# jzr99/Geo4D

Hardware: AMD Instinct MI355X
Metric: denoised latent frames/sec (16x320x512, 50-step DDIM) (higher is better)
Workload: dtype bf16x3m

## Files before the change

### geo4d_amd/_lib.py

```python
import ctypes as C
import os

import torch

_HERE = os.path.dirname(os.path.abspath(__file__))
LIB_PATH = os.environ.get("GEO4D_HIP_LIB") or os.path.join(_HERE, "csrc", "libgeo4d_hip.so")
ABI_VERSION = 9

F32, BF16, F16, BF16X3, F16X2 = 0, 1, 2, 3, 4


class Geo4DNativeError(RuntimeError):
    pass


class ConvGemm(C.Structure):
    _fields_ = [
        ("A", C.c_void_p), ("W", C.c_void_p), ("O", C.c_void_p),
        ("bias", C.c_void_p), ("rowbias", C.c_void_p), ("R", C.c_void_p),
        ("zeros", C.c_void_p), ("workspace", C.c_void_p), ("workspace_bytes", C.c_size_t),
        ("lda", C.c_long), ("ldw", C.c_long), ("ldo", C.c_long), ("ldr", C.c_long), ("ldrb", C.c_long),
        ("a_bs", C.c_long), ("w_bs", C.c_long), ("o_bs", C.c_long), ("r_bs", C.c_long),
        ("M", C.c_int), ("N", C.c_int), ("K", C.c_int), ("batch", C.c_int),
        ("Cin", C.c_int),
# ... 6 lines not shown
        ("a_split", C.c_int), ("w_split", C.c_int), ("o_split", C.c_int), ("gn_colsum", C.c_void_p), ("sat_count", C.c_void_p),
    ]


class GroupNorm(C.Structure):
    _fields_ = [
        ("x", C.c_void_p), ("y", C.c_void_p), ("gamma", C.c_void_p), ("beta", C.c_void_p),
        ("workspace", C.c_void_p), ("workspace_bytes", C.c_size_t),
        ("ldx", C.c_long), ("ldy", C.c_long),
        ("F", C.c_int), ("HW", C.c_int), ("C", C.c_int), ("groups", C.c_int), ("frames_per_stat", C.c_int),
        ("act", C.c_int), ("dtype", C.c_int), ("eps", C.c_float), ("colsum", C.c_void_p), ("split_out", C.c_int), ("colsum_rows", C.c_int),
        ("sat_count", C.c_void_p),
    ]


class Attention(C.Structure):
    _fields_ = [
        ("q", C.c_void_p), ("o", C.c_void_p),
        ("k", C.c_void_p * 2), ("vt", C.c_void_p * 2), ("zeros", C.c_void_p),
        ("ldq", C.c_long), ("ldo", C.c_long), ("ldk", C.c_long * 2), ("ldvt", C.c_long * 2), ("vt_bs", C.c_long * 2),
        ("Nk", C.c_int * 2), ("kv_div", C.c_int * 2),
        ("B", C.c_int), ("H", C.c_int), ("Nq", C.c_int), ("nseg", C.c_int), ("head_dim", C.c_int), ("dtype", C.c_int),
        ("scale", C.c_float), ("split_out", C.c_int), ("variant", C.c_int), ("qkv_split", C.c_int),
    ]


class Align(C.Structure):
    _fields_ = [
        ("pred", C.c_void_p), ("conf", C.c_void_p), ("logdepth", C.c_void_p), ("cams", C.c_void_p), ("slot_trf", C.c_void_p),
        ("slot_ptr", C.c_void_p), ("slot_idx", C.c_void_p),
# ... 16 lines not shown
        ("slot_st", C.c_void_p), ("s_depth", C.c_void_p), ("t_depth", C.c_void_p), ("depth_ok", C.c_void_p),
        ("traj", C.c_void_p), ("traj_align", C.c_void_p), ("traj_valid", C.c_void_p), ("slot_img", C.c_void_p), ("img_slot_ptr", C.c_void_p),
        ("img_slot_idx", C.c_void_p), ("grad_traj", C.c_void_p),
        ("n_imgs", C.c_int), ("n_groups", C.c_int), ("n_slots", C.c_int), ("slots_per_group", C.c_int), ("n_listed_slots", C.c_int),
        ("n_focals", C.c_int), ("norm_pw_scale", C.c_int),
        ("focal_break", C.c_float), ("base_scale", C.c_float), ("ppx", C.c_float), ("ppy", C.c_float), ("smooth_weight", C.c_float),
        ("translation_weight", C.c_float), ("traj_weight", C.c_float),
    ]


SIGNATURES = {
    "geo4d_conv_gemm": (C.c_int, [C.POINTER(ConvGemm), C.c_void_p]),
    "geo4d_conv_gemm_colsum_rows": (C.c_int, [C.POINTER(ConvGemm)]),
    "geo4d_groupnorm_workspace": (C.c_size_t, [C.c_int, C.c_int, C.c_int, C.c_int]),
    "geo4d_groupnorm": (C.c_int, [C.POINTER(GroupNorm), C.c_void_p]),
    "geo4d_layernorm": (C.c_int, [C.c_void_p, C.c_long, C.c_void_p, C.c_long, C.c_int, C.c_int, C.c_float, C.c_void_p,
                                  C.c_void_p, C.c_int, C.c_void_p]),
    "geo4d_layernorm_split": (C.c_int, [C.c_void_p, C.c_long, C.c_void_p, C.c_long, C.c_int, C.c_int, C.c_float, C.c_void_p,
                                        C.c_void_p, C.c_int, C.c_void_p, C.c_void_p]),
    "geo4d_softmax_rows": (C.c_int, [C.c_void_p, C.c_long, C.c_void_p, C.c_long, C.c_long, C.c_int, C.c_float, C.c_int,
                                     C.c_void_p]),
    "geo4d_softmax_rows_causal": (C.c_int, [C.c_void_p, C.c_long, C.c_void_p, C.c_long, C.c_long, C.c_int, C.c_float, C.c_int,
                                            C.c_int, C.c_void_p]),
    "geo4d_attention": (C.c_int, [C.POINTER(Attention), C.c_void_p]),
    "geo4d_temporal_attention": (C.c_int, [C.c_void_p, C.c_long, C.c_void_p, C.c_long, C.c_void_p, C.c_long, C.c_void_p,
                                           C.c_long, C.c_int, C.c_int, C.c_int, C.c_int, C.c_int, C.c_float, C.c_int,
                                           C.c_void_p]),
    "geo4d_temporal_attention2": (C.c_int, [C.c_void_p, C.c_long, C.c_void_p, C.c_long, C.c_void_p, C.c_long, C.c_void_p,
                                            C.c_long, C.c_int, C.c_int, C.c_int, C.c_int, C.c_int, C.c_float, C.c_int,
                                            C.c_int, C.c_void_p]),
# ... 98 lines not shown
```

### geo4d_amd/csrc/norm.hip

```cpp
#include <type_traits>
#include "common.h"
#include "geo4d_hip.h"

namespace {

__host__ __device__ inline int gn_rows_per_chunk(int HW, int F) {
    long r = ((long)HW * F + 1023) / 1024;
    r = (r + 3) / 4 * 4;
    if (r < 4) r = 4;
    if (r > 1024) r = 1024;
    return (int)r;
}

template <typename T>
__device__ __forceinline__ void gn_partial_body(char* smem, const T* __restrict__ x, long ldx, int HW, int C, int G,
                                                int R, int nchunk, float* __restrict__ part, int chunk, int f) {
    constexpr int EPC = Elem<T>::EPC;
    float* stage = (float*)smem;
    float* chs = stage + 256 * 2 * EPC;
    float* chq = chs + C;
    const int tid = threadIdx.x;
    const int CPR = C / EPC;
    const int TC = CPR < 256 ? CPR : 256;
    const int TR = 256 / TC;
// ... 124 lines not shown
    if (tid == 0) {
        s = ((red[0][0] + red[1][0]) + red[2][0]) + red[3][0];
        q = ((red[0][1] + red[1][1]) + red[2][1]) + red[3][1];
        const double n = (double)blocks_per_stat * rows * cpg;
        const double mean = s / n;
        double var = q / n - mean * mean;
        if (var < 0.0) var = 0.0;
        stats[((long)stat * G + grp) * 2 + 0] = (float)mean;
        stats[((long)stat * G + grp) * 2 + 1] = (float)(1.0 / sqrt(var + (double)eps));
    }
}

template <typename T, int SPLIT>
__device__ __forceinline__ void gn_apply_body(const T* __restrict__ x, long ldx, T* __restrict__ y, long ldy,
                                              int HW, int C, int G, int R, const float* st, const float* __restrict__ gamma,
                                              const float* __restrict__ beta, int act, int chunk, int f, unsigned long long* sat) {
    constexpr int EPC = Elem<T>::EPC;
    const int tid = threadIdx.x;
    const int CPR = C / EPC;
    const int TC = CPR < 256 ? CPR : 256;
    const int TR = 256 / TC;
    const int tc = tid % TC, tr = tid / TC;
    if (tr >= TR) return;
    const int row0 = chunk * R;
    const int rows = min(R, HW - row0);
    const int cpg = C / G;
    const T* xb = x + ((long)f * HW + row0) * ldx;
    T* yb = y + ((long)f * HW + row0) * ldy;
    for (int cc = tc; cc < CPR; cc += TC) {
        float sc[EPC], sh[EPC];
#pragma unroll
        for (int j = 0; j < EPC; ++j) {
            const int c = cc * EPC + j;
            const int gi = c / cpg;
            const float mean = st[gi * 2], rstd = st[gi * 2 + 1];
            sc[j] = rstd * gamma[c];
            sh[j] = beta[c] - mean * sc[j];
        }
        for (int r = tr; r < rows; r += 4 * TR) {
            u32x4 v[4];
#pragma unroll
            for (int u = 0; u < 4; ++u) {
                const int ru = r + u * TR;
                v[u] = ru < rows ? *(const u32x4*)(xb + (long)ru * ldx + cc * EPC) : u32x4{0u, 0u, 0u, 0u};
// ... 13 lines not shown
                if constexpr (SPLIT == 1) store_split4(yb + (long)ru * ldy, cc, e);
                else if constexpr (SPLIT == 2) {
                    count_f16_saturation(sat, e);
                    store4_f16((char*)y + ((long)f * HW + row0 + ru) * ldy * 2, cc, e);
                } else *(u32x4*)(yb + (long)ru * ldy + cc * EPC) = f32_to_chunk<T>(e);
            }
        }
    }
}
template <typename T, int SPLIT>
__global__ __launch_bounds__(256) void gn_apply_kernel(const T* __restrict__ x, long ldx, T* __restrict__ y, long ldy,
                                                       int HW, int C, int G, int fps, int R,
                                                       const float* __restrict__ stats, const float* __restrict__ gamma,
                                                       const float* __restrict__ beta, int act, unsigned long long* sat) {
    const int f = blockIdx.y;
    gn_apply_body<T, SPLIT>(x, ldx, y, ldy, HW, C, G, R, stats + (long)(f / fps) * G * 2, gamma, beta, act, blockIdx.x, f, sat);
}

template <typename T, int MAXC, int SPLIT = 0>
__global__ __launch_bounds__(256) void ln_kernel(const T* __restrict__ x, long ldx, T* __restrict__ y, long ldy, int M, int C,
                                                 float eps, const float* __restrict__ gamma, const float* __restrict__ beta, unsigned long long* sat) {
    constexpr int EPC = Elem<T>::EPC;
    const int lane = threadIdx.x & 63;
    const long row = (long)blockIdx.x * 4 + (threadIdx.x >> 6);
    if (row >= M) return;
    const int CPR = C / EPC;
    float e[MAXC][EPC];
    float s = 0.f;
#pragma unroll
    for (int i = 0; i < MAXC; ++i) {
        const int cc = lane + i * 64;
// ... 98 lines not shown
    m = wave_max(m);
    if ((tid & 63) == 0) red[tid >> 6] = m;
    __syncthreads();
    m = fmaxf(fmaxf(red[0], red[1]), fmaxf(red[2], red[3]));
    __syncthreads();
    float s = 0.f;
    for (int c = tid; c < cols; c += 256) s += __expf(xr[c] * scale - m);
    s = wave_sum(s);
    if ((tid & 63) == 0) red[tid >> 6] = s;
    __syncthreads();
    s = (red[0] + red[1]) + (red[2] + red[3]);
    const float inv = 1.0f / s;
    for (int c = tid; c < cols; c += 256) Elem<T>::st(yr + c, __expf(xr[c] * scale - m) * inv);
}

template <typename T, int SPLIT>
int groupnorm_typed(const geo4d_groupnorm_t& p, hipStream_t s) {
    constexpr int EPC = Elem<T>::EPC;
    int R = gn_rows_per_chunk(p.HW, p.F);
    int nchunk = (p.HW + R - 1) / R;
    float* part = (float*)p.workspace;
    const size_t smem = (size_t)256 * 2 * EPC * 4 + (size_t)2 * p.C * 4;
    const int nstat = p.F / p.frames_per_stat;
    float* stats = part + (size_t)p.F * nchunk * p.groups * 3;
    if (p.colsum) {
        const int crows = p.colsum_rows > 0 ? p.colsum_rows : 32;
        hipLaunchKernelGGL(gn_finalize_cols_kernel, dim3(nstat * p.groups), dim3(256), 0, s, p.colsum, (p.frames_per_stat * p.HW) / crows,
                           p.C, p.groups, p.eps, stats, nstat, crows);
        GEO4D_CHECK_LAUNCH();
    } else {
        hipLaunchKernelGGL(gn_partial_kernel<T>, dim3(nchunk, p.F), dim3(256), smem, s, (const T*)p.x, (long)p.ldx, p.HW, p.C, p.groups,
                           R, nchunk, part);
        GEO4D_CHECK_LAUNCH();
        hipLaunchKernelGGL(gn_finalize_kernel, dim3((nstat * p.groups + 3) / 4), dim3(256), 0, s, part, nchunk, p.frames_per_stat,
                           p.groups, p.eps, stats, nstat);
        GEO4D_CHECK_LAUNCH();
    }
    hipLaunchKernelGGL((gn_apply_kernel<T, SPLIT>), dim3(nchunk, p.F), dim3(256), 0, s, (const T*)p.x, (long)p.ldx, (T*)p.y, (long)p.ldy, p.HW,
                       p.C, p.groups, p.frames_per_stat, R, stats, p.gamma, p.beta, p.act, SPLIT == 2 ? p.sat_count : nullptr);
    GEO4D_CHECK_LAUNCH();
    return GEO4D_OK;
}

template <typename T, int SPLIT = 0>
int layernorm_typed(const void* x, long ldx, void* y, long ldy, int M, int C, float eps, const float* g, const float* b,
                    hipStream_t s, unsigned long long* sat = nullptr) {
    constexpr int EPC = Elem<T>::EPC;
    if constexpr (std::is_same<T, float>::value) {
        const bool al = ((uintptr_t)g % 16) == 0 && ((uintptr_t)b % 16) == 0;
        const dim3 grid16((M + 15) / 16);
#define LN16_LAUNCH(NC) hipLaunchKernelGGL((ln16_kernel<NC, SPLIT>), grid16, dim3(256), 0, s, (const float*)x, ldx, (float*)y, ldy, M, eps, g, b, sat)
        if (al && C == 320) { LN16_LAUNCH(5); GEO4D_CHECK_LAUNCH(); return GEO4D_OK; }
        if (al && C == 640) { LN16_LAUNCH(10); GEO4D_CHECK_LAUNCH(); return GEO4D_OK; }
#undef LN16_LAUNCH
// ... 3 lines not shown
#define LN_LAUNCH(MC) hipLaunchKernelGGL((ln_kernel<T, MC, SPLIT>), grid, dim3(256), 0, s, (const T*)x, ldx, (T*)y, ldy, M, C, eps, g, b, sat)
    if (per_lane <= 1) LN_LAUNCH(1);
    else if (per_lane <= 2) LN_LAUNCH(2);
    else if (per_lane <= 3) LN_LAUNCH(3);
    else if (per_lane <= 5) LN_LAUNCH(5);
    else if (per_lane <= 10) LN_LAUNCH(10);
    else { geo4d_set_error("layernorm: C too large"); return GEO4D_ENOTSUP; }
#undef LN_LAUNCH
    GEO4D_CHECK_LAUNCH();
    return GEO4D_OK;
}

}

extern "C" size_t geo4d_groupnorm_workspace(int F, int HW, int groups, int frames_per_stat) {
    const int R = gn_rows_per_chunk(HW, F);
    const int nchunk = (HW + R - 1) / R;
    return ((size_t)F * nchunk * groups * 3 + (size_t)(F / frames_per_stat) * groups * 2) * sizeof(float);
}

extern "C" int geo4d_groupnorm(const geo4d_groupnorm_t* pp, void* stream) {
    if (!pp) return GEO4D_EINVAL;
    const geo4d_groupnorm_t& p = *pp;
    const int esz = p.dtype == GEO4D_F32 ? 4 : 2, epc = 16 / esz;
    if (p.dtype < 0 || p.dtype > 2) { geo4d_set_error("groupnorm: bad dtype"); return GEO4D_EINVAL; }
    if (p.F <= 0 || p.HW <= 0 || p.C <= 0 || p.groups <= 0 || p.groups > 32 || p.C % p.groups || p.C % epc) {
        geo4d_set_error("groupnorm: need C % groups == 0, C % (16 B) == 0, groups <= 32");
        return GEO4D_EINVAL;
    }
    if (p.frames_per_stat <= 0 || p.F % p.frames_per_stat) { geo4d_set_error("groupnorm: F % frames_per_stat"); return GEO4D_EINVAL; }
    const int yesz = p.split_out == 2 ? 2 : esz;
    if ((p.ldx * esz) % 16 || (p.ldy * yesz) % 16 || ((uintptr_t)p.x % 16) || ((uintptr_t)p.y % 16)) { geo4d_set_error("groupnorm: alignment"); return GEO4D_EINVAL; }
    if (p.workspace_bytes < geo4d_groupnorm_workspace(p.F, p.HW, p.groups, p.frames_per_stat)) { geo4d_set_error("groupnorm: workspace too small"); return GEO4D_EINVAL; }
    if (p.F > 65535) { geo4d_set_error("groupnorm: too many frames"); return GEO4D_EINVAL; }
    {
        const int crows = p.colsum_rows > 0 ? p.colsum_rows : 32;
        if (p.colsum && ((((long)p.frames_per_stat * p.HW) % crows) || ((uintptr_t)p.colsum % 8))) {
            geo4d_set_error("groupnorm: colsum needs (frames_per_stat x HW) % colsum_rows == 0");
            return GEO4D_EINVAL;
        }
    }
    if (p.split_out && (p.dtype != GEO4D_F32 || (p.C % 8) || p.split_out > 2 || p.split_out < 0)) { geo4d_set_error("groupnorm: split_out (1 = bf16 hi | lo, 2 = plain f16 rows) is a producer format for f32 input, C % 8 == 0"); return GEO4D_EINVAL; }
    hipStream_t s = (hipStream_t)stream;
    switch (p.dtype) {
        case GEO4D_F32: return p.split_out == 2 ? groupnorm_typed<float, 2>(p, s) : p.split_out ? groupnorm_typed<float, 1>(p, s) : groupnorm_typed<float, 0>(p, s);
        case GEO4D_BF16: return groupnorm_typed<bf16_t, 0>(p, s);
        default: return groupnorm_typed<f16_t, 0>(p, s);
    }
}

extern "C" int geo4d_layernorm(const void* x, long ldx, void* y, long ldy, int M, int C, float eps, const float* gamma,
                               const float* beta, int dtype, void* stream) {
    const int esz = dtype == GEO4D_F32 ? 4 : 2, epc = 16 / esz;
    if (dtype < 0 || dtype > 2 || M <= 0 || C <= 0 || C % epc || (ldx * esz) % 16 || (ldy * esz) % 16 || ((uintptr_t)x % 16) || ((uintptr_t)y % 16)) {
        geo4d_set_error("layernorm: bad arguments");
        return GEO4D_EINVAL;
    }
    hipStream_t s = (hipStream_t)stream;
    switch (dtype) {
        case GEO4D_F32: return layernorm_typed<float>(x, ldx, y, ldy, M, C, eps, gamma, beta, s);
        case GEO4D_BF16: return layernorm_typed<bf16_t>(x, ldx, y, ldy, M, C, eps, gamma, beta, s);
        default: return layernorm_typed<f16_t>(x, ldx, y, ldy, M, C, eps, gamma, beta, s);
    }
// ... 37 lines not shown
```

### geo4d_amd/ops.py

```python
import ctypes as C

import torch

from . import _lib
from ._lib import BF16, BF16X3, F16, F16X2, F32, Attention, ConvGemm, GroupNorm
from .precision import resolve as _resolve_precision

_DT = {torch.float32: F32, torch.bfloat16: BF16, torch.float16: F16}
_TD = {F32: torch.float32, BF16: torch.bfloat16, F16: torch.float16}


def dt_code(dtype):
    try:
        return _DT[dtype]
    except KeyError:
        raise TypeError(f"geo4d_amd: unsupported dtype {dtype} (float32, bfloat16, float16 only)")


def k_align(dtype):
    return 32 if _resolve_precision(dtype).storage == torch.float32 else 64


class X2Weight(torch.Tensor):
    _KEEP = {"to", "clone", "detach", "contiguous", "cuda", "cpu", "pin_memory"}
# ... 105 lines not shown


AUTOTUNE = _os.environ.get("GEO4D_AUTOTUNE", "1") != "0"
def _env_level(name, default):
    v = _os.environ.get(name)
    if v is None or not v.strip():
        return default
    v = v.strip().lower()
    try:
        return int(v)
    except ValueError:
        return 0 if v in ("off", "false", "no", "none") else 1


GN_FUSED_STATS = _env_level("GEO4D_GN_FUSED", 1)
SPLITK_COLSUM = _env_level("GEO4D_SPLITK_COLSUM", 1)
TUNE_EXACT = _env_level("GEO4D_TUNE_EXACT", 0)
TUNE_LOG = []
DEBUG_ABLATE = _env_level("GEO4D_DEBUG_ABLATE", 0)
GEMM_TIMELINE = None
ATTN_TIMELINE = None
SAT_COUNTER = None


def _tune_table():
    global _TUNE
    if _TUNE is None:
        _TUNE = {}
        if _os.path.exists(_TUNE_PATH):
            with open(_TUNE_PATH) as f:
# ... 238 lines not shown
    if out is None:
        out = torch.empty((M, N), device=x.device, dtype=_out_dtype(x, None, w))
    return conv_gemm(x, w, out, M=M, N=N, K=3 * Cin, Cin=Cin, lda=_ld(x), ldw=_ld(w), ldo=_ld(out), T=T, Hin=HW, Win=1,
                     Hout=HW, Wout=1, KT=3, pt=1, bias=bias, residual=residual,
                     ldr=_ld(residual) if residual is not None else 0, gn_stats=gn_stats, tile_hint=tile_hint, split_k=split_k)


def batched_gemm(a, b, out, *, batch, M, N, K, a_bs, b_bs, o_bs, bias=None, bias_per_row=False, alpha=1.0, x3=False):
    return conv_gemm(a, b, out, M=M, N=N, K=K, Cin=K, lda=_ld(a), ldw=_ld(b), ldo=_ld(out), batch=batch, a_bs=a_bs,
                     w_bs=b_bs, o_bs=o_bs, bias=bias, bias_per_row=bias_per_row, alpha=alpha, x3=x3)


_gn_ws = {}


def groupnorm(x, gamma, beta, *, F, HW, eps, groups=32, frames_per_stat=1, silu=False, out=None, split_out=False):
    lib = _lib.load()
    _dev(x, "x")
    assert not isinstance(x, SplitAct), "GroupNorm reads plain activations"
    Cc = x.shape[1]
    assert x.shape[0] == F * HW, (x.shape, F, HW)
    assert gamma.dtype == torch.float32 and beta.dtype == torch.float32
    if out is None:
        out = new_split(F * HW, Cc, x.device, split_fmt(split_out)[1]) if split_out else torch.empty((F * HW, Cc), device=x.device, dtype=x.dtype)
    split_out = 1 if isinstance(out, SplitAct) else 2 if (out.dtype == torch.float16 and x.dtype == torch.float32) else 0
    if split_out:
        assert x.dtype == torch.float32, "the GEMM-operand producer formats are written from f32 activations"
    if split_out == 1:
        _split_out_ok(out, F * HW)
    need = lib.geo4d_groupnorm_workspace(F, HW, groups, frames_per_stat)
    ws = torch.empty(need, device=x.device, dtype=torch.uint8)
    p = GroupNorm()
    p.x, p.y, p.gamma, p.beta = x.data_ptr(), out.data_ptr(), gamma.data_ptr(), beta.data_ptr()
    p.workspace, p.workspace_bytes = ws.data_ptr(), need
    p.ldx, p.ldy = _ld(x), (_ld(out) // 2 if split_out == 1 else _ld(out))
    p.split_out = int(split_out)
    p.sat_count = _ptr(SAT_COUNTER) if split_out == 2 else 0
    p.F, p.HW, p.C, p.groups, p.frames_per_stat = F, HW, Cc, groups, frames_per_stat
    p.act, p.dtype, p.eps = int(silu), dt_code(x.dtype), eps
    cs = getattr(x, "_gn_colsum", None)
    if cs is not None and getattr(x, "_gn_colsum_tag", None) != (x.data_ptr(), x._version):
        cs = None
    rows = getattr(x, "_gn_colsum_rows", 32)
    ok = cs is not None and (frames_per_stat * HW) % rows == 0 and tuple(cs.shape) == (F * HW // rows, Cc, 2)
    p.colsum, p.colsum_rows = (cs.data_ptr(), rows) if ok else (0, 0)
    _lib.check(lib.geo4d_groupnorm(C.byref(p), _stream()), "geo4d_groupnorm")
    return out


def layernorm(x, gamma, beta, eps=1e-5, out=None, split_out=False):
    lib = _lib.load()
    _dev(x, "x")
    assert not isinstance(x, SplitAct), "LayerNorm reads plain activations"
    M, Cc = x.shape
    if split_out or isinstance(out, SplitAct) or (out is not None and out.dtype == torch.float16 and x.dtype == torch.float32):
        assert x.dtype == torch.float32
        if out is None:
            out = new_split(M, Cc, x.device, split_fmt(split_out)[1])
        if isinstance(out, SplitAct):
            _split_out_ok(out, M)
            _lib.check(lib.geo4d_layernorm_split(x.data_ptr(), _ld(x), out.data_ptr(), _ld(out) // 2, M, Cc, eps, gamma.data_ptr(),
# ... 514 lines not shown
```

### geo4d_amd/unet.py

```python
import math
import os

import torch
import torch.nn as nn

from . import ops, pack
from .precision import resolve as resolve_dtype


class ParamTree(nn.Module):

    def __init__(self):
        super().__init__()

    def insert(self, dotted, shape):
        node = self
        parts = dotted.split(".")
        for part in parts[:-1]:
            child = node._modules.get(part)
            if child is None:
                child = ParamTree()
                node.add_module(part, child)
            node = child
        node.register_parameter(parts[-1], nn.Parameter(torch.empty(shape), requires_grad=False))
# ... 489 lines not shown
        t_emb = ops.timestep_embedding(timesteps.to(torch.int64), P["freqs"])
        w0, b0, w2, b2 = P["time"]
        emb = ops.linear_small(ops.linear_small(t_emb, w0, b0, act_out=True), w2, b2)
        if self.fs_condition:
            if fs is None:
                fs = torch.full((B,), self.default_fs, dtype=torch.int64, device=x.device)
            w0, b0, w2, b2 = P["fps"]
            f_emb = ops.timestep_embedding(fs.to(torch.int64), P["freqs"])
            emb = ops.linear_small(ops.linear_small(f_emb, w0, b0, act_out=True), w2, b2, add=emb)
        emb_all = ops.linear_small(emb, P["emb_w"], P["emb_b"], act_in=True)
        kv = self._context_kv(P, context, B, T)
        e0 = P[inputs[0][0].prefix]
        h = ops.tokens_from_ncthw(x.float().contiguous(), None if c_concat is None else c_concat.float().contiguous(), e0["cpad"], dt)
        n_in = len(inputs)
        cats = {}

        def half(j, left):
            if not FUSED_CONCAT or j >= len(outputs):
                return None
            ccat = outputs[j][0].cin

            def view(rows, j=j, left=left, ccat=ccat):
                buf = cats.get(j)
                if buf is None:
                    buf = cats[j] = torch.empty((rows, ccat), device=x.device, dtype=dt)
                assert buf.shape[0] == rows, "latent height/width must be multiples of 8"
                cs = skip_ch[n_in - 1 - j]
                return buf[:, :ccat - cs] if left else buf[:, ccat - cs:]
            return view
        skip_ch = [blk[-1].cout if blk[-1].kind != "temporal" and blk[-1].kind != "spatial" else blk[-1].cin for blk in inputs]
        o0 = half(n_in - 1, False)
        if init_attn is not None:
            h, _, _ = ops.conv2d(h, e0["w"], e0["b"], F=B * T, Hin=H, Win=W, KH=3, KW=3, pad=1, gn_stats=True)
            h = self._temporal(P[init_attn.prefix], init_attn, h, B, T, H, W, out=None if o0 is None else o0(B * T * H * W))
        else:
            h, _, _ = ops.conv2d(h, e0["w"], e0["b"], F=B * T, Hin=H, Win=W, KH=3, KW=3, pad=1, gn_stats=True, out=None if o0 is None else o0(B * T * H * W))
        hs = [(h, H, W)]
        for i, blk in enumerate(inputs[1:], start=1):
            h, H, W = self._run(P, blk, h, emb_all, kv, B, T, H, W, out=half(n_in - 1 - i, False))
            hs.append((h, H, W))
        h, H, W = self._run(P, middle, h, emb_all, kv, B, T, H, W, out=half(0, True))
        for j, blk in enumerate(outputs):
            s, sh, sw = hs.pop()
# ... 8 lines not shown
```

### include/geo4d_hip.h

```cpp
#ifndef GEO4D_HIP_H
#define GEO4D_HIP_H
#include <stddef.h>
#ifdef __cplusplus
extern "C" {
#endif

#define GEO4D_ABI_VERSION 9

typedef struct geo4d_conv_gemm_t {
    const void* A;
    const void* W;
    void* O;
    const float* bias;
    const float* rowbias;
    const void* R;
    const void* zeros;
    void* workspace;
    size_t workspace_bytes;
    long lda, ldw, ldo, ldr;
    long ldrb;
    long a_bs, w_bs, o_bs, r_bs;
    int M, N, K, batch;
    int Cin;
    int T, Hin, Win, Hout, Wout;
// ... 21 lines not shown
    const float* gamma; const float* beta;
    void* workspace; size_t workspace_bytes;
    long ldx, ldy;
    int F, HW, C, groups, frames_per_stat;
    int act;
    int dtype;
    float eps;
    const float* colsum;
    int split_out;
    int colsum_rows;
    unsigned long long* sat_count;
} geo4d_groupnorm_t;
size_t geo4d_groupnorm_workspace(int F, int HW, int groups, int frames_per_stat);
int geo4d_groupnorm(const geo4d_groupnorm_t* p, void* stream);

int geo4d_layernorm(const void* x, long ldx, void* y, long ldy, int M, int C, float eps, const float* gamma,
                    const float* beta, int dtype, void* stream);

int geo4d_layernorm_split(const void* x, long ldx, void* y, long ldy, int M, int C, float eps, const float* gamma,
                          const float* beta, int fmt, unsigned long long* sat_count, void* stream);

int geo4d_softmax_rows(const float* x, long ldx, void* y, long ldy, long rows, int cols, float scale, int out_dtype,
                       void* stream);
int geo4d_softmax_rows_causal(const float* x, long ldx, void* y, long ldy, long rows, int cols, float scale, int out_dtype,
                              int causal_period, void* stream);

typedef struct geo4d_attention_t {
    const void* q; void* o;
    const void* k[2]; const void* vt[2];
    const void* zeros;
// ... 123 lines not shown
```

Before: 6.822.

## Add planned GroupNorm paths fusing column-sum statistics into the apply kernel

Adds a GroupNorm2 descriptor and planner that can fold the statistics finalization into the apply kernel: each workgroup reduces the producer's column sums for its groups and then normalizes, giving a single launch. It can also use a sliced two-launch path. Column sums from both halves of a fused concat buffer are passed as two sources, so GroupNorm after a skip concat can skip the separate partial-stats pass. The cost is redundant reduction of the column sums in every workgroup, which the planner bounds by sizing chunks and channel slices. It also adds planner complexity and a per-call plan query from the host.

```diff
diff --git a/geo4d_amd/_lib.py b/geo4d_amd/_lib.py
--- a/geo4d_amd/_lib.py
+++ b/geo4d_amd/_lib.py
@@ -44,6 +44,23 @@
     ]
 
 
+class GroupNormSrc(C.Structure):
+    _fields_ = [("colsum", C.c_void_p), ("rows", C.c_int), ("c0", C.c_int), ("channels", C.c_int)]
+
+
+class GroupNorm2(C.Structure):
+    _fields_ = [("base", GroupNorm), ("src", GroupNormSrc * 2), ("nsrc", C.c_int), ("path", C.c_int), ("fuse_fraction", C.c_float),
+                ("min_workgroups", C.c_int)]
+
+
+class GroupNormPlan(C.Structure):
+    _fields_ = [("path", C.c_int), ("launches", C.c_int), ("rows_per_wg", C.c_int), ("nchunk", C.c_int), ("channel_slices", C.c_int),
+                ("stat_slices", C.c_int), ("workspace_bytes", C.c_size_t)]
+
+
+GN_PATH_AUTO, GN_PATH_PARTIAL, GN_PATH_COLS, GN_PATH_FUSED, GN_PATH_SLICED = 0, 1, 2, 3, 4
+
+
 class Attention(C.Structure):
     _fields_ = [
         ("q", C.c_void_p), ("o", C.c_void_p),
@@ -90,6 +107,8 @@
     "geo4d_conv_gemm_colsum_rows": (C.c_int, [C.POINTER(ConvGemm)]),
     "geo4d_groupnorm_workspace": (C.c_size_t, [C.c_int, C.c_int, C.c_int, C.c_int]),
     "geo4d_groupnorm": (C.c_int, [C.POINTER(GroupNorm), C.c_void_p]),
+    "geo4d_groupnorm_plan": (C.c_int, [C.POINTER(GroupNorm2), C.POINTER(GroupNormPlan)]),
+    "geo4d_groupnorm2": (C.c_int, [C.POINTER(GroupNorm2), C.c_void_p]),
     "geo4d_layernorm": (C.c_int, [C.c_void_p, C.c_long, C.c_void_p, C.c_long, C.c_int, C.c_int, C.c_float, C.c_void_p,
                                   C.c_void_p, C.c_int, C.c_void_p]),
     "geo4d_layernorm_split": (C.c_int, [C.c_void_p, C.c_long, C.c_void_p, C.c_long, C.c_int, C.c_int, C.c_float, C.c_void_p,
diff --git a/geo4d_amd/csrc/norm.hip b/geo4d_amd/csrc/norm.hip
--- a/geo4d_amd/csrc/norm.hip
+++ b/geo4d_amd/csrc/norm.hip
@@ -162,10 +162,11 @@
 template <typename T, int SPLIT>
 __device__ __forceinline__ void gn_apply_body(const T* __restrict__ x, long ldx, T* __restrict__ y, long ldy,
                                               int HW, int C, int G, int R, const float* st, const float* __restrict__ gamma,
-                                              const float* __restrict__ beta, int act, int chunk, int f, unsigned long long* sat) {
+                                              const float* __restrict__ beta, int act, int chunk, int f, unsigned long long* sat,
+                                              int cbeg, int cend) {
     constexpr int EPC = Elem<T>::EPC;
     const int tid = threadIdx.x;
-    const int CPR = C / EPC;
+    const int CPR = cend - cbeg;
     const int TC = CPR < 256 ? CPR : 256;
     const int TR = 256 / TC;
     const int tc = tid % TC, tr = tid / TC;
@@ -175,7 +176,7 @@
     const int cpg = C / G;
     const T* xb = x + ((long)f * HW + row0) * ldx;
     T* yb = y + ((long)f * HW + row0) * ldy;
-    for (int cc = tc; cc < CPR; cc += TC) {
+    for (int cc = cbeg + tc; cc < cend; cc += TC) {
         float sc[EPC], sh[EPC];
 #pragma unroll
         for (int j = 0; j < EPC; ++j) {
@@ -219,7 +220,99 @@
                                                        const float* __restrict__ stats, const float* __restrict__ gamma,
                                                        const float* __restrict__ beta, int act, unsigned long long* sat) {
     const int f = blockIdx.y;
-    gn_apply_body<T, SPLIT>(x, ldx, y, ldy, HW, C, G, R, stats + (long)(f / fps) * G * 2, gamma, beta, act, blockIdx.x, f, sat);
+    gn_apply_body<T, SPLIT>(x, ldx, y, ldy, HW, C, G, R, stats + (long)(f / fps) * G * 2, gamma, beta, act, blockIdx.x, f, sat, 0, C / Elem<T>::EPC);
+}
+
+struct GnSrc { const float* cs; int nb, c0, nc; };
+struct GnSums { GnSrc s[2]; int nsrc; };
+
+__device__ __forceinline__ void gn_sum_items(const GnSrc& S, int stat, int b0, int b1, int ca, int cb, int l, int ts, double& s, double& q) {
+    const int lo = max(ca, S.c0), hi = min(cb, S.c0 + S.nc);
+    const int nch = hi - lo;
+    if (nch <= 0 || b1 <= b0) return;
+    const int total = (b1 - b0) * nch;
+    const float* base = S.cs + (((long)stat * S.nb + b0) * S.nc + (lo - S.c0)) * 2;
+    for (int i = l; i < total; i += 4 * ts) {
+        f32x2 v[4];
+#pragma unroll
+        for (int u = 0; u < 4; ++u) {
+            const int iu = i + u * ts;
+            v[u] = f32x2{0.f, 0.f};
+            if (iu < total) {
+                const int rb = iu / nch, c = iu - rb * nch;
+                v[u] = *(const f32x2*)(base + ((long)rb * S.nc + c) * 2);
+            }
+        }
+#pragma unroll
+        for (int u = 0; u < 4; ++u) { s += (double)v[u][0]; q += (double)v[u][1]; }
+    }
+}
+__device__ __forceinline__ void gn_mean_rstd(double s, double q, double n, float eps, float* st) {
+    const double mean = s / n;
+    double var = q / n - mean * mean;
+    if (var < 0.0) var = 0.0;
+    st[0] = (float)mean;
+    st[1] = (float)(1.0 / sqrt(var + (double)eps));
+}
+
+__global__ __launch_bounds__(256) void gn_slice_sums_kernel(GnSums S, int C, int G, int ns, double* __restrict__ part) {
+    __shared__ double red[4][2];
+    const int tid = threadIdx.x, lane = tid & 63, wave = tid >> 6;
+    const int unit = blockIdx.x / ns, k = blockIdx.x - unit * ns;
+    const int stat = unit / G, grp = unit - stat * G;
+    const int cpg = C / G;
+    double s = 0.0, q = 0.0;
+    for (int i = 0; i < S.nsrc; ++i) {
+        const int b0 = (int)((long)k * S.s[i].nb / ns), b1 = (int)((long)(k + 1) * S.s[i].nb / ns);
+        gn_sum_items(S.s[i], stat, b0, b1, grp * cpg, (grp + 1) * cpg, tid, 256, s, q);
+    }
+#pragma unroll
+    for (int o = 1; o < 64; o <<= 1) {
+        s += __shfl_xor(s, o);
+        q += __shfl_xor(q, o);
+    }
+    if (lane == 0) { red[wave][0] = s; red[wave][1] = q; }
+    __syncthreads();
+    if (tid == 0) {
+        part[(long)blockIdx.x * 2 + 0] = ((red[0][0] + red[1][0]) + red[2][0]) + red[3][0];
+        part[(long)blockIdx.x * 2 + 1] = ((red[0][1] + red[1][1]) + red[2][1]) + red[3][1];
+    }
+}
+
+template <typename T, int SPLIT>
+__global__ __launch_bounds__(256) void gn_apply_sums_kernel(const T* __restrict__ x, long ldx, T* __restrict__ y, long ldy,
+                                                            int HW, int C, int G, int fps, int R, int ncs, GnSums S, int ns,
+                                                            const double* __restrict__ part, float eps, const float* __restrict__ gamma,
+                                                            const float* __restrict__ beta, int act, unsigned long long* sat) {
+    __shared__ float st[64];
+    const int tid = threadIdx.x;
+    const int f = blockIdx.y, stat = f / fps;
+    const int cpg = C / G, gps = G / ncs, g0 = blockIdx.z * gps;
+    const double n = (double)fps * HW * cpg;
+    if (ns == 0) {
+        int ts = 64;
+        while (ts * gps > 256) ts >>= 1;
+        const int team = tid / ts, l = tid - team * ts;
+        double s = 0.0, q = 0.0;
+        if (team < gps) {
+            const int g = g0 + team;
+            for (int i = 0; i < S.nsrc; ++i) gn_sum_items(S.s[i], stat, 0, S.s[i].nb, g * cpg, (g + 1) * cpg, l, ts, s, q);
+        }
+        for (int o = 1; o < ts; o <<= 1) {
+            s += __shfl_xor(s, o);
+            q += __shfl_xor(q, o);
+        }
+        if (team < gps && l == 0) gn_mean_rstd(s, q, n, eps, st + (g0 + team) * 2);
+    } else if (tid < gps) {
+        const int g = g0 + tid;
+        const double* pp = part + ((long)stat * G + g) * ns * 2;
+        double s = 0.0, q = 0.0;
+        for (int k = 0; k < ns; ++k) { s += pp[k * 2]; q += pp[k * 2 + 1]; }
+        gn_mean_rstd(s, q, n, eps, st + g * 2);
+    }
+    __syncthreads();
+    constexpr int EPC = Elem<T>::EPC;
+    gn_apply_body<T, SPLIT>(x, ldx, y, ldy, HW, C, G, R, st, gamma, beta, act, blockIdx.x, f, sat, g0 * cpg / EPC, (g0 + gps) * cpg / EPC);
 }
 
 template <typename T, int MAXC, int SPLIT = 0>
@@ -348,18 +441,143 @@
     for (int c = tid; c < cols; c += 256) Elem<T>::st(yr + c, __expf(xr[c] * scale - m) * inv);
 }
 
+constexpr float GN_FUSE_FRACTIONS[2] = {0.125f, 0.25f};
+constexpr int GN_MIN_WORKGROUPS = 1024;
+constexpr size_t GN_FUSE_MAX_TRAFFIC = (size_t)12 << 20;
+constexpr int GN_MAX_STAT_SLICES = 64;
+
+inline int gn_stat_slices(int nstat, int G) {
+    int ns = (256 + nstat * G - 1) / (nstat * G);
+    return ns < 1 ? 1 : ns > GN_MAX_STAT_SLICES ? GN_MAX_STAT_SLICES : ns;
+}
+inline size_t gn_workspace_partial(int F, int HW, int G, int fps) {
+    const int R = gn_rows_per_chunk(HW, F);
+    const int nchunk = (HW + R - 1) / R;
+    return ((size_t)F * nchunk * G * 3 + (size_t)(F / fps) * G * 2) * sizeof(float);
+}
+
+int gn_plan(const geo4d_groupnorm2_t& q, geo4d_groupnorm_plan_t& o) {
+    const geo4d_groupnorm_t& p = q.base;
+    o = geo4d_groupnorm_plan_t{};
+    if (p.dtype < 0 || p.dtype > 2) { geo4d_set_error("groupnorm: bad dtype"); return GEO4D_EINVAL; }
+    const int esz = p.dtype == GEO4D_F32 ? 4 : 2, epc = 16 / esz;
+    if (p.F <= 0 || p.HW <= 0 || p.C <= 0 || p.groups <= 0 || p.groups > 32 || p.C % p.groups || p.C % epc) {
+        geo4d_set_error("groupnorm: need C % groups == 0, C % (16 B) == 0, groups <= 32");
+        return GEO4D_EINVAL;
+    }
+    if (p.frames_per_stat <= 0 || p.F % p.frames_per_stat) { geo4d_set_error("groupnorm: F % frames_per_stat"); return GEO4D_EINVAL; }
+    const int yesz = p.split_out == 2 ? 2 : esz;
+    if ((p.ldx * esz) % 16 || (p.ldy * yesz) % 16 || ((uintptr_t)p.x % 16) || ((uintptr_t)p.y % 16)) { geo4d_set_error("groupnorm: alignment"); return GEO4D_EINVAL; }
+    if (p.F > 65535) { geo4d_set_error("groupnorm: too many frames"); return GEO4D_EINVAL; }
+    if (p.split_out && (p.dtype != GEO4D_F32 || (p.C % 8) || p.split_out > 2 || p.split_out < 0)) { geo4d_set_error("groupnorm: split_out (1 = bf16 hi | lo, 2 = plain f16 rows) is a producer format for f32 input, C % 8 == 0"); return GEO4D_EINVAL; }
+    if (q.nsrc < 0 || q.nsrc > 2 || q.path < 0 || q.path > GEO4D_GN_PATH_SLICED || !(q.fuse_fraction >= 0.f) || q.min_workgroups < 0) {
+        geo4d_set_error("groupnorm: bad nsrc / path / fuse_fraction / min_workgroups");
+        return GEO4D_EINVAL;
+    }
+    const long stat_rows = (long)p.frames_per_stat * p.HW;
+    int cnext = 0;
+    size_t sum_bytes = 0;
+    int max_nb = 1;
+    for (int i = 0; i < q.nsrc; ++i) {
+        const geo4d_groupnorm_src_t& r = q.src[i];
+        if (!r.colsum || ((uintptr_t)r.colsum % 8) || r.rows <= 0 || (stat_rows % r.rows)) {
+            geo4d_set_error("groupnorm: colsum needs (frames_per_stat x HW) % colsum_rows == 0");
+            return GEO4D_EINVAL;
+        }
+        if (r.c0 != cnext || r.channels <= 0) { geo4d_set_error("groupnorm: the sum sources must tile the channels in order"); return GEO4D_EINVAL; }
+        cnext += r.channels;
+        const int nb = (int)(stat_rows / r.rows);
+        sum_bytes += (size_t)nb * r.channels * 8;
+        if (nb > max_nb) max_nb = nb;
+    }
+    if (q.nsrc && cnext != p.C) { geo4d_set_error("groupnorm: the sum sources must tile the channels in order"); return GEO4D_EINVAL; }
+    if (!q.nsrc && (q.path == GEO4D_GN_PATH_FUSED || q.path == GEO4D_GN_PATH_SLICED)) { geo4d_set_error("groupnorm: this path needs column sums"); return GEO4D_EINVAL; }
+
+    const int G = p.groups, cpg = p.C / G, nstat = p.F / p.frames_per_stat;
+    const int R0 = gn_rows_per_chunk(p.HW, p.F), nchunk0 = (p.HW + R0 - 1) / R0;
+    o.rows_per_wg = R0; o.nchunk = nchunk0; o.channel_slices = 1; o.stat_slices = 0;
+    if (!q.nsrc || q.path == GEO4D_GN_PATH_PARTIAL || (q.path == GEO4D_GN_PATH_COLS && q.nsrc != 1)) {
+        o.path = GEO4D_GN_PATH_PARTIAL; o.launches = 3;
+        o.workspace_bytes = gn_workspace_partial(p.F, p.HW, G, p.frames_per_stat);
+        return GEO4D_OK;
+    }
+    if (q.path == GEO4D_GN_PATH_COLS) {
+        o.path = GEO4D_GN_PATH_COLS; o.launches = 2;
+        o.workspace_bytes = gn_workspace_partial(p.F, p.HW, G, p.frames_per_stat);
+        return GEO4D_OK;
+    }
+    if (q.path != GEO4D_GN_PATH_SLICED) {
+        const long minwg = q.min_workgroups > 0 ? q.min_workgroups : GN_MIN_WORKGROUPS;
+        const long floor_wg = (long)p.F * nchunk0 < minwg ? (long)p.F * nchunk0 : minwg;
+        const double row_bytes = (double)p.C * (esz + yesz);
+        const long HWr = ((long)p.HW + 3) / 4 * 4;
+        const int nfrac = q.fuse_fraction > 0.f ? 1 : 2;
+        for (int fi = 0; fi < nfrac; ++fi) {
+            const float frac = q.fuse_fraction > 0.f ? q.fuse_fraction : GN_FUSE_FRACTIONS[fi];
+            long R = (long)((double)sum_bytes / ((double)frac * row_bytes) + 0.999999);
+            if (R < R0) R = R0;
+            R = (R + 3) / 4 * 4;
+            if (R > HWr && R != R0) continue;
+            const int nchunk = (int)((p.HW + R - 1) / R);
+            if (!q.path && !(q.fuse_fraction > 0.f) && (size_t)p.F * nchunk * sum_bytes > GN_FUSE_MAX_TRAFFIC) continue;
+            for (int ncs = 1; ncs <= G; ++ncs) {
+                if (G % ncs) continue;
+                const int cslice = G / ncs * cpg;
+                if (cslice % epc || (ncs > 1 && cslice * esz < 256)) continue;
+                if ((long)p.F * nchunk * ncs < floor_wg) continue;
+                o.path = GEO4D_GN_PATH_FUSED; o.launches = 1;
+                o.rows_per_wg = (int)R; o.nchunk = nchunk; o.channel_slices = ncs;
+                o.workspace_bytes = 0;
+                return GEO4D_OK;
+            }
+        }
+        if (q.path == GEO4D_GN_PATH_FUSED) {
+            o.path = GEO4D_GN_PATH_FUSED; o.launches = 1; o.workspace_bytes = 0;
+            return GEO4D_OK;
+        }
+    }
+    if (!q.path && q.nsrc == 1 && gn_stat_slices(nstat, G) == 1) {
+        o.path = GEO4D_GN_PATH_COLS; o.launches = 2;
+        o.workspace_bytes = gn_workspace_partial(p.F, p.HW, G, p.frames_per_stat);
+        return GEO4D_OK;
+    }
+    o.path = GEO4D_GN_PATH_SLICED; o.launches = 2;
+    o.stat_slices = gn_stat_slices(nstat, G);
+    if (o.stat_slices > max_nb) o.stat_slices = max_nb;
+    o.workspace_bytes = (size_t)nstat * G * o.stat_slices * 2 * sizeof(double);
+    if ((uintptr_t)p.workspace % 8) { geo4d_set_error("groupnorm: workspace alignment"); return GEO4D_EINVAL; }
+    return GEO4D_OK;
+}
+
 template <typename T, int SPLIT>
-int groupnorm_typed(const geo4d_groupnorm_t& p, hipStream_t s) {
+int groupnorm_typed(const geo4d_groupnorm2_t& q, const geo4d_groupnorm_plan_t& pl, hipStream_t s) {
     constexpr int EPC = Elem<T>::EPC;
-    int R = gn_rows_per_chunk(p.HW, p.F);
-    int nchunk = (p.HW + R - 1) / R;
+    const geo4d_groupnorm_t& p = q.base;
+    const int nstat = p.F / p.frames_per_stat;
+    unsigned long long* sat = SPLIT == 2 ? p.sat_count : nullptr;
+    if (pl.path == GEO4D_GN_PATH_FUSED || pl.path == GEO4D_GN_PATH_SLICED) {
+        GnSums S{};
+        S.nsrc = q.nsrc;
+        for (int i = 0; i < q.nsrc; ++i)
+            S.s[i] = GnSrc{q.src[i].colsum, (int)(((long)p.frames_per_stat * p.HW) / q.src[i].rows), q.src[i].c0, q.src[i].channels};
+        double* part = (double*)p.workspace;
+        if (pl.path == GEO4D_GN_PATH_SLICED) {
+            hipLaunchKernelGGL(gn_slice_sums_kernel, dim3(nstat * p.groups * pl.stat_slices), dim3(256), 0, s, S, p.C, p.groups, pl.stat_slices, part);
+            GEO4D_CHECK_LAUNCH();
+        }
+        hipLaunchKernelGGL((gn_apply_sums_kernel<T, SPLIT>), dim3(pl.nchunk, p.F, pl.channel_slices), dim3(256), 0, s, (const T*)p.x, (long)p.ldx,
+                           (T*)p.y, (long)p.ldy, p.HW, p.C, p.groups, p.frames_per_stat, pl.rows_per_wg, pl.channel_slices, S, pl.stat_slices,
+                           part, p.eps, p.gamma, p.beta, p.act, sat);
+        GEO4D_CHECK_LAUNCH();
+        return GEO4D_OK;
+    }
+    const int R = pl.rows_per_wg, nchunk = pl.nchunk;
     float* part = (float*)p.workspace;
     const size_t smem = (size_t)256 * 2 * EPC * 4 + (size_t)2 * p.C * 4;
-    const int nstat = p.F / p.frames_per_stat;
     float* stats = part + (size_t)p.F * nchunk * p.groups * 3;
-    if (p.colsum) {
-        const int crows = p.colsum_rows > 0 ? p.colsum_rows : 32;
-        hipLaunchKernelGGL(gn_finalize_cols_kernel, dim3(nstat * p.groups), dim3(256), 0, s, p.colsum, (p.frames_per_stat * p.HW) / crows,
+    if (pl.path == GEO4D_GN_PATH_COLS) {
+        const int crows = q.src[0].rows;
+        hipLaunchKernelGGL(gn_finalize_cols_kernel, dim3(nstat * p.groups), dim3(256), 0, s, q.src[0].colsum, (p.frames_per_stat * p.HW) / crows,
                            p.C, p.groups, p.eps, stats, nstat, crows);
         GEO4D_CHECK_LAUNCH();
     } else {
@@ -371,7 +589,7 @@
         GEO4D_CHECK_LAUNCH();
     }
     hipLaunchKernelGGL((gn_apply_kernel<T, SPLIT>), dim3(nchunk, p.F), dim3(256), 0, s, (const T*)p.x, (long)p.ldx, (T*)p.y, (long)p.ldy, p.HW,
-                       p.C, p.groups, p.frames_per_stat, R, stats, p.gamma, p.beta, p.act, SPLIT == 2 ? p.sat_count : nullptr);
+                       p.C, p.groups, p.frames_per_stat, R, stats, p.gamma, p.beta, p.act, sat);
     GEO4D_CHECK_LAUNCH();
     return GEO4D_OK;
 }
@@ -405,39 +623,49 @@
 }
 
 extern "C" size_t geo4d_groupnorm_workspace(int F, int HW, int groups, int frames_per_stat) {
-    const int R = gn_rows_per_chunk(HW, F);
-    const int nchunk = (HW + R - 1) / R;
-    return ((size_t)F * nchunk * groups * 3 + (size_t)(F / frames_per_stat) * groups * 2) * sizeof(float);
+    const size_t a = gn_workspace_partial(F, HW, groups, frames_per_stat);
+    const size_t b = (size_t)(F / frames_per_stat) * groups * gn_stat_slices(F / frames_per_stat, groups) * 2 * sizeof(double);
+    return a > b ? a : b;
+}
+
+extern "C" int geo4d_groupnorm_plan(const geo4d_groupnorm2_t* q, geo4d_groupnorm_plan_t* plan) {
+    if (!q || !plan) return GEO4D_EINVAL;
+    return gn_plan(*q, *plan);
+}
+
+extern "C" int geo4d_groupnorm2(const geo4d_groupnorm2_t* qq, void* stream) {
+    if (!qq) return GEO4D_EINVAL;
+    const geo4d_groupnorm2_t& q = *qq;
+    const geo4d_groupnorm_t& p = q.base;
+    geo4d_groupnorm_plan_t pl;
+    const int rc = gn_plan(q, pl);
+    if (rc != GEO4D_OK) return rc;
+    if (p.workspace_bytes < pl.workspace_bytes || (pl.workspace_bytes && !p.workspace)) { geo4d_set_error("groupnorm: workspace too small"); return GEO4D_EINVAL; }
+    hipStream_t s = (hipStream_t)stream;
+    switch (p.dtype) {
+        case GEO4D_F32: return p.split_out == 2 ? groupnorm_typed<float, 2>(q, pl, s) : p.split_out ? groupnorm_typed<float, 1>(q, pl, s) : groupnorm_typed<float, 0>(q, pl, s);
+        case GEO4D_BF16: return groupnorm_typed<bf16_t, 0>(q, pl, s);
+        default: return groupnorm_typed<f16_t, 0>(q, pl, s);
+    }
 }
 
 extern "C" int geo4d_groupnorm(const geo4d_groupnorm_t* pp, void* stream) {
     if (!pp) return GEO4D_EINVAL;
-    const geo4d_groupnorm_t& p = *pp;
-    const int esz = p.dtype == GEO4D_F32 ? 4 : 2, epc = 16 / esz;
-    if (p.dtype < 0 || p.dtype > 2) { geo4d_set_error("groupnorm: bad dtype"); return GEO4D_EINVAL; }
-    if (p.F <= 0 || p.HW <= 0 || p.C <= 0 || p.groups <= 0 || p.groups > 32 || p.C % p.groups || p.C % epc) {
-        geo4d_set_error("groupnorm: need C % groups == 0, C % (16 B) == 0, groups <= 32");
+    geo4d_groupnorm2_t q{};
+    q.base = *pp;
+    if (pp->colsum) {
+        q.nsrc = 1;
+        q.src[0] = geo4d_groupnorm_src_t{pp->colsum, pp->colsum_rows > 0 ? pp->colsum_rows : 32, 0, pp->C};
+    }
+    if (pp->workspace_bytes < geo4d_groupnorm_workspace(pp->F > 0 ? pp->F : 1, pp->HW > 0 ? pp->HW : 1, pp->groups > 0 ? pp->groups : 1,
+                                                        pp->frames_per_stat > 0 ? pp->frames_per_stat : 1)) {
+        geo4d_groupnorm_plan_t pl;
+        const int rc = gn_plan(q, pl);
+        if (rc != GEO4D_OK) return rc;
+        geo4d_set_error("groupnorm: workspace too small");
         return GEO4D_EINVAL;
     }
-    if (p.frames_per_stat <= 0 || p.F % p.frames_per_stat) { geo4d_set_error("groupnorm: F % frames_per_stat"); return GEO4D_EINVAL; }
-    const int yesz = p.split_out == 2 ? 2 : esz;
-    if ((p.ldx * esz) % 16 || (p.ldy * yesz) % 16 || ((uintptr_t)p.x % 16) || ((uintptr_t)p.y % 16)) { geo4d_set_error("groupnorm: alignment"); return GEO4D_EINVAL; }
-    if (p.workspace_bytes < geo4d_groupnorm_workspace(p.F, p.HW, p.groups, p.frames_per_stat)) { geo4d_set_error("groupnorm: workspace too small"); return GEO4D_EINVAL; }
-    if (p.F > 65535) { geo4d_set_error("groupnorm: too many frames"); return GEO4D_EINVAL; }
-    {
-        const int crows = p.colsum_rows > 0 ? p.colsum_rows : 32;
-        if (p.colsum && ((((long)p.frames_per_stat * p.HW) % crows) || ((uintptr_t)p.colsum % 8))) {
-            geo4d_set_error("groupnorm: colsum needs (frames_per_stat x HW) % colsum_rows == 0");
-            return GEO4D_EINVAL;
-        }
-    }
-    if (p.split_out && (p.dtype != GEO4D_F32 || (p.C % 8) || p.split_out > 2 || p.split_out < 0)) { geo4d_set_error("groupnorm: split_out (1 = bf16 hi | lo, 2 = plain f16 rows) is a producer format for f32 input, C % 8 == 0"); return GEO4D_EINVAL; }
-    hipStream_t s = (hipStream_t)stream;
-    switch (p.dtype) {
-        case GEO4D_F32: return p.split_out == 2 ? groupnorm_typed<float, 2>(p, s) : p.split_out ? groupnorm_typed<float, 1>(p, s) : groupnorm_typed<float, 0>(p, s);
-        case GEO4D_BF16: return groupnorm_typed<bf16_t, 0>(p, s);
-        default: return groupnorm_typed<f16_t, 0>(p, s);
-    }
+    return geo4d_groupnorm2(&q, stream);
 }
 
 extern "C" int geo4d_layernorm(const void* x, long ldx, void* y, long ldy, int M, int C, float eps, const float* gamma,
diff --git a/geo4d_amd/ops.py b/geo4d_amd/ops.py
--- a/geo4d_amd/ops.py
+++ b/geo4d_amd/ops.py
@@ -3,7 +3,7 @@
 import torch
 
 from . import _lib
-from ._lib import BF16, BF16X3, F16, F16X2, F32, Attention, ConvGemm, GroupNorm
+from ._lib import BF16, BF16X3, F16, F16X2, F32, Attention, ConvGemm, GroupNorm2, GroupNormPlan
 from .precision import resolve as _resolve_precision
 
 _DT = {torch.float32: F32, torch.bfloat16: BF16, torch.float16: F16}
@@ -143,6 +143,8 @@
 
 
 GN_FUSED_STATS = _env_level("GEO4D_GN_FUSED", 1)
+GN_ONE_LAUNCH = _env_level("GEO4D_GN_ONE_LAUNCH", 1)
+GN_TUNE = (0.0, 0)
 SPLITK_COLSUM = _env_level("GEO4D_SPLITK_COLSUM", 1)
 TUNE_EXACT = _env_level("GEO4D_TUNE_EXACT", 0)
 TUNE_LOG = []
@@ -411,7 +413,63 @@
 _gn_ws = {}
 
 
-def groupnorm(x, gamma, beta, *, F, HW, eps, groups=32, frames_per_stat=1, silu=False, out=None, split_out=False):
+def _gn_sums(t, stat_rows):
+    cs = getattr(t, "_gn_colsum", None)
+    if cs is None or getattr(t, "_gn_colsum_tag", None) != (t.data_ptr(), t._version):
+        return None
+    rows = getattr(t, "_gn_colsum_rows", 32)
+    if stat_rows % rows or tuple(cs.shape) != (t.shape[0] // rows, t.shape[1], 2):
+        return None
+    return cs, rows
+
+
+def concat_parts(buf, left, right):
+    buf._gn_parts = (left, right)
+
+
+def _gn_sources(x, stat_rows):
+    one = _gn_sums(x, stat_rows)
+    if one is not None:
+        return [(one[0], one[1], 0, x.shape[1])]
+    parts = getattr(x, "_gn_parts", None)
+    if not parts or not GN_ONE_LAUNCH:
+        return []
+    src, c0 = [], 0
+    for v in parts:
+        if v.dim() != 2 or v.shape[0] != x.shape[0] or v.stride() != x.stride() or v.data_ptr() != x.data_ptr() + c0 * x.element_size():
+            return []
+        sums = _gn_sums(v, stat_rows)
+        if sums is None:
+            return []
+        src.append((sums[0], sums[1], c0, v.shape[1]))
+        c0 += v.shape[1]
+    return src if c0 == x.shape[1] else []
+
+
+def _gn_descriptor(x, out, gamma, beta, *, F, HW, eps, groups, frames_per_stat, silu, split_out, sources, path):
+    q = GroupNorm2()
+    p = q.base
+    p.x, p.y, p.gamma, p.beta = x.data_ptr(), out.data_ptr(), gamma.data_ptr(), beta.data_ptr()
+    p.ldx, p.ldy = _ld(x), (_ld(out) // 2 if split_out == 1 else _ld(out))
+    p.split_out = int(split_out)
+    p.sat_count = _ptr(SAT_COUNTER) if split_out == 2 else 0
+    p.F, p.HW, p.C, p.groups, p.frames_per_stat = F, HW, x.shape[1], groups, frames_per_stat
+    p.act, p.dtype, p.eps = int(silu), dt_code(x.dtype), eps
+    q.nsrc = len(sources)
+    for i, (cs, rows, c0, nc) in enumerate(sources):
+        q.src[i].colsum, q.src[i].rows, q.src[i].c0, q.src[i].channels = cs.data_ptr(), rows, c0, nc
+    q.path = path
+    q.fuse_fraction, q.min_workgroups = GN_TUNE
+    return q
+
+
+def groupnorm_plan(q):
+    plan = GroupNormPlan()
+    _lib.check(_lib.load().geo4d_groupnorm_plan(C.byref(q), C.byref(plan)), "geo4d_groupnorm_plan")
+    return plan
+
+
+def groupnorm(x, gamma, beta, *, F, HW, eps, groups=32, frames_per_stat=1, silu=False, out=None, split_out=False, path=None):
     lib = _lib.load()
     _dev(x, "x")
     assert not isinstance(x, SplitAct), "GroupNorm reads plain activations"
@@ -425,23 +483,18 @@
         assert x.dtype == torch.float32, "the GEMM-operand producer formats are written from f32 activations"
     if split_out == 1:
         _split_out_ok(out, F * HW)
-    need = lib.geo4d_groupnorm_workspace(F, HW, groups, frames_per_stat)
-    ws = torch.empty(need, device=x.device, dtype=torch.uint8)
-    p = GroupNorm()
-    p.x, p.y, p.gamma, p.beta = x.data_ptr(), out.data_ptr(), gamma.data_ptr(), beta.data_ptr()
-    p.workspace, p.workspace_bytes = ws.data_ptr(), need
-    p.ldx, p.ldy = _ld(x), (_ld(out) // 2 if split_out == 1 else _ld(out))
-    p.split_out = int(split_out)
-    p.sat_count = _ptr(SAT_COUNTER) if split_out == 2 else 0
-    p.F, p.HW, p.C, p.groups, p.frames_per_stat = F, HW, Cc, groups, frames_per_stat
-    p.act, p.dtype, p.eps = int(silu), dt_code(x.dtype), eps
-    cs = getattr(x, "_gn_colsum", None)
-    if cs is not None and getattr(x, "_gn_colsum_tag", None) != (x.data_ptr(), x._version):
-        cs = None
-    rows = getattr(x, "_gn_colsum_rows", 32)
-    ok = cs is not None and (frames_per_stat * HW) % rows == 0 and tuple(cs.shape) == (F * HW // rows, Cc, 2)
-    p.colsum, p.colsum_rows = (cs.data_ptr(), rows) if ok else (0, 0)
-    _lib.check(lib.geo4d_groupnorm(C.byref(p), _stream()), "geo4d_groupnorm")
+    if path is None:
+        path = {0: _lib.GN_PATH_COLS, 3: _lib.GN_PATH_FUSED, 4: _lib.GN_PATH_SLICED}.get(int(GN_ONE_LAUNCH), _lib.GN_PATH_AUTO)
+    sources = _gn_sources(x, frames_per_stat * HW)
+    if not sources:
+        path = _lib.GN_PATH_PARTIAL
+    q = _gn_descriptor(x, out, gamma, beta, F=F, HW=HW, eps=eps, groups=groups, frames_per_stat=frames_per_stat, silu=silu,
+                       split_out=split_out, sources=sources, path=path)
+    need = groupnorm_plan(q).workspace_bytes
+    if need:
+        ws = torch.empty(need, device=x.device, dtype=torch.uint8)
+        q.base.workspace, q.base.workspace_bytes = ws.data_ptr(), need
+    _lib.check(lib.geo4d_groupnorm2(C.byref(q), _stream()), "geo4d_groupnorm2")
     return out
 
 
diff --git a/geo4d_amd/unet.py b/geo4d_amd/unet.py
--- a/geo4d_amd/unet.py
+++ b/geo4d_amd/unet.py
@@ -527,6 +527,7 @@
         h = ops.tokens_from_ncthw(x.float().contiguous(), None if c_concat is None else c_concat.float().contiguous(), e0["cpad"], dt)
         n_in = len(inputs)
         cats = {}
+        halves = {}
 
         def half(j, left):
             if not FUSED_CONCAT or j >= len(outputs):
@@ -539,7 +540,11 @@
                     buf = cats[j] = torch.empty((rows, ccat), device=x.device, dtype=dt)
                 assert buf.shape[0] == rows, "latent height/width must be multiples of 8"
                 cs = skip_ch[n_in - 1 - j]
-                return buf[:, :ccat - cs] if left else buf[:, ccat - cs:]
+                v = buf[:, :ccat - cs] if left else buf[:, ccat - cs:]
+                halves[(j, left)] = v
+                if (j, True) in halves and (j, False) in halves:
+                    ops.concat_parts(buf, halves[(j, True)], halves[(j, False)])
+                return v
             return view
         skip_ch = [blk[-1].cout if blk[-1].kind != "temporal" and blk[-1].kind != "spatial" else blk[-1].cin for blk in inputs]
         o0 = half(n_in - 1, False)
diff --git a/include/geo4d_hip.h b/include/geo4d_hip.h
--- a/include/geo4d_hip.h
+++ b/include/geo4d_hip.h
@@ -59,6 +59,37 @@
 size_t geo4d_groupnorm_workspace(int F, int HW, int groups, int frames_per_stat);
 int geo4d_groupnorm(const geo4d_groupnorm_t* p, void* stream);
 
+typedef struct geo4d_groupnorm_src_t {
+    const float* colsum;
+    int rows;
+    int c0, channels;
+} geo4d_groupnorm_src_t;
+typedef struct geo4d_groupnorm2_t {
+    geo4d_groupnorm_t base;
+    geo4d_groupnorm_src_t src[2];
+    int nsrc;
+    int path;
+    float fuse_fraction;
+    int min_workgroups;
+} geo4d_groupnorm2_t;
+enum {
+    GEO4D_GN_PATH_PARTIAL = 1,
+    GEO4D_GN_PATH_COLS = 2,
+    GEO4D_GN_PATH_FUSED = 3,
+    GEO4D_GN_PATH_SLICED = 4
+};
+typedef struct geo4d_groupnorm_plan_t {
+    int path;
+    int launches;
+    int rows_per_wg;
+    int nchunk;
+    int channel_slices;
+    int stat_slices;
+    size_t workspace_bytes;
+} geo4d_groupnorm_plan_t;
+int geo4d_groupnorm_plan(const geo4d_groupnorm2_t* p, geo4d_groupnorm_plan_t* plan);
+int geo4d_groupnorm2(const geo4d_groupnorm2_t* p, void* stream);
+
 int geo4d_layernorm(const void* x, long ldx, void* y, long ldy, int M, int C, float eps, const float* gamma,
                     const float* beta, int dtype, void* stream);
 
```

After: 6.903, median of 6. +1.2%, better.
